# LepistaBioinformatics/classeq2

Hardware: AMD Instinct MI355X
Metric: query placements/sec, 10k-leaf tree, 150 bp reads (higher is better)
Workload: dtype u64

## Files before the change

classeq2_amd/csrc/cls_api.cpp:

```cpp
#include <hip/hip_runtime.h>
#include <ctype.h>
#include <stdio.h>
#include <stdlib.h>
#include <string.h>

#include <algorithm>
#include <mutex>
#include <new>
#include <string>
#include <thread>
#include <vector>

#include "cls_db.h"
#include "cls_device.h"
#include "cls_kernels.h"
#include "cls_place.h"
#include "cls_tally.h"
#include "cls_tuning.h"

namespace {

thread_local std::string g_err;

int fail(int code, const std::string& msg) {
// ... 74 lines not shown
    std::vector<CallSlot> calls;
    struct TreeRow { uint64_t id; uint32_t pre, size; };
    std::vector<TreeRow> tree_rows;
};

namespace cls {
Tuning& tuning() {
    static Tuning t;
    return t;
}
}
namespace {
struct Knob { const char* name; int cls::Tuning::*field; };
const Knob KNOBS[] = {
    {"no_fast", &cls::Tuning::no_fast}, {"no_order", &cls::Tuning::no_order}, {"force_list", &cls::Tuning::force_list},
    {"no_mask_halves", &cls::Tuning::no_mask_halves}, {"no_fat_direct", &cls::Tuning::no_fat_direct}, {"no_tile", &cls::Tuning::no_tile}, {"tile_pass_codes", &cls::Tuning::tile_pass_codes}, {"tile_set_words", &cls::Tuning::tile_set_words}, {"time_class", &cls::Tuning::time_class}, {"tile_one_per_cu", &cls::Tuning::tile_one_per_cu}, {"tile_min_kmers", &cls::Tuning::tile_min_kmers}, {"no_tile_order", &cls::Tuning::no_tile_order}, {"tile_deal", &cls::Tuning::tile_deal}, {"blocks_per_cu", &cls::Tuning::blocks_per_cu}, {"key_blocks_per_cu", &cls::Tuning::key_blocks_per_cu},
    {"long_blocks_per_cu", &cls::Tuning::long_blocks_per_cu}, {"order_mode", &cls::Tuning::order_mode},
    {"order_windows", &cls::Tuning::order_windows}, {"order_both_strands", &cls::Tuning::order_both_strands},
    {"order_block_shift", &cls::Tuning::order_block_shift}, {"order_sample_shift", &cls::Tuning::order_sample_shift},
    {"profile_stop", &cls::Tuning::profile_stop}, {"timing", &cls::Tuning::timing},
    {"build_full_key", &cls::Tuning::build_full_key}, {"tally_no_wave_combine", &cls::Tuning::tally_no_wave_combine},
};
}

extern "C" int cls_set_tuning(const char* name, int value) {
    if (!name) return fail(CLS_E_INVALID_ARG, "cls_set_tuning: null name");
    for (const Knob& k : KNOBS)
        if (strcmp(k.name, name) == 0) { cls::tuning().*(k.field) = value; return CLS_OK; }
    return fail(CLS_E_INVALID_ARG, std::string("cls_set_tuning: unknown knob ") + name);
}

// ... 102 lines not shown
    v.mz_bucket = (const uint32_t*)db->d_mz_bucket;
    v.direct = (const uint32_t*)db->d_direct;
    v.direct16 = (const uint32_t*)db->d_direct16;
    v.sets = (const cls::SetRec*)db->d_sets;
    v.sets2 = (const cls::SetRec*)db->d_sets2;
    v.table_mask = E.table.size() - 1;
    v.n_nodes = (uint32_t)E.nodes.size();
    v.n_buckets = (uint32_t)E.bucket_key.size();
    v.k = E.k;
    v.m_eff = E.m_eff;
    v.max_nonleaf_arity = E.max_nonleaf_arity;
    v.format = E.format;
    v.binary_tree = E.strictly_binary ? 1u : 0u;
    v.canonical = E.canonical ? 1u : 0u;
    v.n_sets = (uint32_t)E.sets.size();
    v.set_bits = 1;
    while (v.set_bits < 32 && (1ull << v.set_bits) < (uint64_t)E.sets.size()) ++v.set_bits;
    v.addr32 = (E.postings.size() * 4 < (1ull << 32) && E.direct.size() * 4 < (1ull << 32) && E.sets.size() * sizeof(cls::SetRec) < (1ull << 32)) ? 1u : 0u;
    cls_db_info& i = db->info;
    i.n_nodes = v.n_nodes;
    i.max_depth = E.max_depth;
    i.max_nonleaf_arity = E.max_nonleaf_arity;
    i.k_size = E.k;
    i.m_size = E.m;
    i.n_buckets = n_buckets;
    i.n_kmers = E.n_kmers;
    i.n_closed_kmers = E.n_closed;
    i.table_slots = E.table.size();
    i.postings_words = E.postings.size();
    i.hbm_bytes = E.nodes.size() * sizeof(cls::DNode) + E.table.size() * sizeof(cls::Slot) + (E.postings.size() + E.postings2.size()) * 4 + E.bucket_key.size() * 8 + E.mz_bucket.size() * 4 + E.direct.size() * 4 + E.direct16.size() * 4 + (E.sets.size() + E.sets2.size()) * sizeof(cls::SetRec);
// ... 998 lines not shown
```

classeq2_amd/csrc/cls_db.cpp:

```cpp
#include "cls_db.h"

#include "cls_murmur.h"
#include "cls_tuning.h"

#include <stdio.h>
#include <stdlib.h>
#include <string.h>

#include <algorithm>
#include <atomic>
#include <chrono>
#include <exception>
#include <functional>
#include <mutex>
#include <thread>

namespace cls {

namespace {

struct WorkerError {
    std::mutex mu;
    std::exception_ptr first;
    void capture() { std::lock_guard<std::mutex> g(mu); if (!first) first = std::current_exception(); }
// ... 336 lines not shown
        parallel_chunks(NK, nt, [&](unsigned, uint64_t lo, uint64_t hi) {
            for (uint64_t j = lo; j < hi; ++j) set_of[j] = rank[tmp_set[j]] + 1;
        });
        std::vector<uint32_t>().swap(tmp_set);
        std::vector<uint32_t>().swap(rank);
        E.n_sets = NS;
        lap("set order");
        std::vector<uint64_t> set_rec(NS + 1);
        uint64_t n_recs = 1;
        for (uint64_t g = 0; g < NS; ++g) { set_rec[g] = n_recs; n_recs += keys[g].n ? keys[g].n - 1 : 0; }
        set_rec[NS] = n_recs;
        if (n_recs >= (1ULL << 32)) { err = "split trees exceed 2^32 records"; return CLS_E_BAD_DB; }
        HugeVec<uint32_t> recs((n_recs + 1) * 4, 0);
        recs[2] = 0xFFFFFFFFu;
        const bool mask_halves = !tuning().no_mask_halves;
        HugeVec<uint32_t> recs2(mask_halves ? (n_recs + 1) * 4 : 0, 0);
        if (mask_halves) { recs2[2] = 0xFFFFFFFFu; set_mask.assign(NS + 1, 0u); }
        E.sets.assign(NS + 1, SetRec{0u, 0xFFFFFFFFu, 0u, 0u});
        parallel_chunks(NS, nt, [&](unsigned, uint64_t lo, uint64_t hi) {
            std::vector<uint32_t> dd, stk, L, R, pos, span_lo, span_hi;
            for (uint64_t g = lo; g < hi; ++g) {
                const uint32_t* w = words_of(keys[g].rep);
                const uint32_t n = w[0] & POST_LEN_MASK;
                const uint32_t* tip = w + POST_HEADER_WORDS;
                const uint64_t base = set_rec[g];
                dd.assign(n, 0); L.assign(n, 0); R.assign(n, 0);
                for (uint32_t i = 1; i < n; ++i) {
                    uint32_t a = tip[i - 1];
                    while (!(tip[i] < a + size_by_pre[a])) a = parent_pre[a];
                    dd[i] = depth_by_pre[a];
// ... 23 lines not shown
                        if (left_heavy) { if (r) stk.push_back(r); if (l) stk.push_back(l); }
                        else { if (l) stk.push_back(l); if (r) stk.push_back(r); }
                    }
                }
                auto at = [&](uint32_t i) { return (uint32_t)(base + pos[i]); };
                for (uint32_t i = 1; i < n; ++i) {
                    uint32_t* t = &recs[(size_t)at(i) * 4];
                    t[0] = tip[i - 1];
                    t[1] = L[i] ? at(L[i]) : 0;
                    t[2] = tip[i];
                    t[3] = R[i] ? at(R[i]) : 0;
                    if (mask_halves) {
                        uint32_t* u = &recs2[(size_t)at(i) * 4];
                        u[0] = t[0]; u[1] = t[1]; u[2] = t[2]; u[3] = t[3];
                        const uint32_t l0 = span_lo[i], r1 = span_hi[i];
                        if (tip[i - 1] - tip[l0] < MASK_HALF_SPAN) {
                            uint32_t bits = 0;
                            for (uint32_t j = l0; j < i; ++j) bits |= 1u << (tip[j] - tip[l0]);
                            u[0] = tip[i - 1] | MASK_HALF; u[1] = bits;
                        }
                        if (tip[r1 - 1] - tip[i] < MASK_HALF_SPAN) {
                            uint32_t bits = 0;
                            for (uint32_t j = i; j < r1; ++j) bits |= 1u << (tip[j] - tip[i]);
                            u[2] = tip[i] | MASK_HALF; u[3] = bits;
                        }
                    }
                }
                if (mask_halves && n && tip[n - 1] - tip[0] < MASK_HALF_SPAN) {
                    uint32_t bits = 0;
                    for (uint32_t j = 0; j < n; ++j) bits |= 1u << (tip[j] - tip[0]);
                    set_mask[g + 1] = bits;
                }
                uint32_t lg = 0;
                while (lg < 31 && (1u << lg) <= n) ++lg;
                SetRec& sr = E.sets[g + 1];
                sr.x = root ? at(root) : 0;
                sr.vlo_lg = n ? ((lg << DIRECT_TIP_BITS) | tip[0]) : 0xFFFFFFFFu;
                sr.vhi_root = (n ? tip[n - 1] : 0u) | ((w[0] & POST_HAS_ROOT) ? 0x80000000u : 0u);
                sr.n_leaf = w[1];
// ... 127 lines not shown
                if (it != by_key.end()) E.mz_bucket[code] = it->second;
            }
        }
    }
    E.k = (uint32_t)d->k_size;
    E.m = (uint32_t)std::min<uint64_t>(d->m_size, UINT32_MAX);
    E.m_eff = (uint32_t)std::min<uint64_t>(d->m_size, d->k_size);
    E.n_kmers = NK;
    E.n_closed = n_closed.load();
    E.root_has_children = d->nodes[0].has_children != 0;
    return CLS_OK;
}

}

extern "C" int cls_db_debug_mask_halves(const cls_db_desc* d, uint64_t* counts) {
    try {
        cls::EncodedDb E;
        std::string err;
        const int rc = cls::encode_db(d, E, err);
        if (rc != CLS_OK) return rc;
        using namespace cls;
        counts[0] = counts[1] = counts[2] = 0;
        if (E.format != FMT_SPLIT || E.postings2.empty()) return CLS_OK;
        if (E.postings2.size() != E.postings.size()) return CLS_E_INTERNAL;
        const TipRec* recs = reinterpret_cast<const TipRec*>(E.postings.data());
        const TipRec* rec2 = reinterpret_cast<const TipRec*>(E.postings2.data());
        const uint64_t n_recs = E.postings.size() / 4;
        std::function<void(uint32_t, uint32_t, int, std::vector<uint32_t>&)> part = [&](uint32_t end_tip, uint32_t x, int side, std::vector<uint32_t>& out) {
            if (!x) { out.push_back(end_tip); return; }
            const TipRec& t = recs[x];
            part(t.tip_prev, t.l, 0, out);
            part(t.tip, t.r, 1, out);
            (void)side;
        };
        std::vector<uint32_t> tips;
        for (uint64_t x = 1; x + 1 < n_recs; ++x) {
            const TipRec& t = recs[x];
            const TipRec& u = rec2[x];
            if (t.tip_prev == 0 && t.tip == 0 && t.l == 0 && t.r == 0) continue;
            ++counts[0];
            for (int side = 0; side < 2; ++side) {
                const uint32_t end_tip = side ? t.tip : t.tip_prev, sub = side ? t.r : t.l;
                const uint32_t uw = side ? u.tip : u.tip_prev, ux = side ? u.r : u.l;
                tips.clear();
                part(end_tip, sub, side, tips);
                if (!std::is_sorted(tips.begin(), tips.end()) || (side ? tips.front() : tips.back()) != end_tip) return CLS_E_INTERNAL;
                const bool narrow = tips.back() - tips.front() < MASK_HALF_SPAN;
                if (uw & MASK_HALF) {
                    uint32_t bits = 0;
                    for (uint32_t v : tips) bits |= 1u << (v - tips.front());
                    if (!narrow || (uw & ~MASK_HALF) != end_tip || ux != bits) return CLS_E_INTERNAL;
                    ++counts[1];
                } else {
                    if (narrow || uw != end_tip || ux != sub) return CLS_E_INTERNAL;
                    ++counts[2];
                }
            }
        }
        return CLS_OK;
    } catch (const std::bad_alloc&) {
        return CLS_E_NOMEM;
    } catch (...) {
        return CLS_E_INTERNAL;
    }
}

extern "C" int cls_db_debug_members(const cls_db_desc* d, const uint64_t* hashes, const uint64_t* clade_ids, uint64_t n, uint8_t* out) {
    try {
        cls::EncodedDb E;
        std::string err;
        const int rc = cls::encode_db(d, E, err);
        if (rc != CLS_OK) return rc;
        using namespace cls;
        std::vector<std::pair<uint64_t, uint32_t>> id2row(E.nodes.size());
        for (uint32_t r = 0; r < E.nodes.size(); ++r) id2row[r] = {E.nodes[r].id, r};
        std::sort(id2row.begin(), id2row.end());
        const uint64_t mask = E.table.size() - 1;
        std::vector<uint32_t> tips, stk;
        for (uint64_t i = 0; i < n; ++i) {
            auto it = std::lower_bound(id2row.begin(), id2row.end(), std::make_pair(clade_ids[i], (uint32_t)0));
// ... 55 lines not shown
```

classeq2_amd/csrc/cls_db.h:

```cpp
#pragma once
#include <stdlib.h>
#include <sys/mman.h>

#include <new>
#include <string>
#include <vector>

#include "cls_device.h"

namespace cls {

constexpr uint64_t MAX_K = 1024;

template <class T>
struct HugeAlloc {
    using value_type = T;
    HugeAlloc() = default;
    template <class U> HugeAlloc(const HugeAlloc<U>&) {}
    T* allocate(size_t n) {
        const size_t bytes = n * sizeof(T);
        if (bytes < (8u << 20)) { void* p = malloc(bytes ? bytes : 1); if (!p) throw std::bad_alloc(); return static_cast<T*>(p); }
        const size_t huge = 2u << 20, padded = (bytes + huge - 1) & ~(huge - 1);
        void* p = aligned_alloc(huge, padded);
        if (!p) throw std::bad_alloc();
// ... 13 lines not shown
    HugeVec<Slot> table;
    HugeVec<uint32_t> postings2;
    HugeVec<uint32_t> postings;
    uint32_t format = FMT_LIST;
    bool strictly_binary = false;
    bool canonical = false;
    std::vector<uint64_t> bucket_key;
    std::vector<uint32_t> mz_bucket;
    HugeVec<SetRec> sets;
    HugeVec<SetRec> sets2;
    HugeVec<uint32_t> direct;
    HugeVec<uint32_t> direct16;
    uint32_t k = 0, m = 0, m_eff = 0;
    uint32_t max_depth = 0, max_nonleaf_arity = 0;
    uint64_t n_kmers = 0, n_closed = 0;
    uint64_t n_sets = 0;
    bool root_has_children = false;
};

int encode_db(const cls_db_desc* d, EncodedDb& E, std::string& err);

}
```

classeq2_amd/csrc/cls_device.h:

```cpp
#pragma once
#include <stdint.h>

#include "cls_place.h"

namespace cls {

struct DNode {
    uint32_t pre;
    uint32_t size;
    uint32_t first_child;
    uint32_t n_nonleaf;
    uint64_t id;
    uint32_t split;
    uint32_t flags;
};
static_assert(sizeof(DNode) == 32, "DNode");

struct Slot {
    uint64_t hash;
    uint64_t loc;
};
static_assert(sizeof(Slot) == 16, "Slot");
constexpr uint64_t SLOT_EMPTY = ~0ULL;
struct TSlot {
// ... 22 lines not shown
};
static_assert(sizeof(SetRec) == 16, "SetRec");
constexpr uint32_t DIRECT_MAX_K = 15;
constexpr uint32_t FAT_DIRECT_MAX_K = 12;
constexpr uint32_t DIRECT_TIP_BITS = 27;
constexpr uint32_t DIRECT_TIP_MASK = (1u << DIRECT_TIP_BITS) - 1;
struct TipRec {
    uint32_t tip_prev;
    uint32_t l;
    uint32_t tip;
    uint32_t r;
};
static_assert(sizeof(TipRec) == 16, "TipRec");
constexpr uint32_t MASK_HALF = 0x80000000u;
constexpr uint32_t MASK_HALF_SPAN = 32;
constexpr uint32_t FAT_X_IS_BITS = 0x40000000u;

enum : uint32_t { FMT_LIST = 0, FMT_SPLIT = 1 };

struct DbDev {
    const DNode* nodes;
    const uint32_t* kids;
    const Slot* table;
    const uint32_t* postings;
    const uint32_t* postings2;
    const uint64_t* bucket_key;
    const uint32_t* mz_bucket;
    const uint32_t* direct;
    const uint32_t* direct16;
    const SetRec* sets;
    const SetRec* sets2;
    uint64_t table_mask;
    uint32_t n_nodes;
    uint32_t n_buckets;
    uint32_t k;
    uint32_t m_eff;
    uint32_t max_nonleaf_arity;
    uint32_t format;
    uint32_t addr32;
    uint32_t binary_tree;
    uint32_t canonical;
    uint32_t set_bits;
    uint32_t n_sets;
};

struct PlaceParams {
    int32_t max_iterations;
    uint32_t remove_intersection;
    double min_match_coverage;
};

constexpr uint32_t MAX_READ_KMERS = 64 * 8 * 16;

}
```

classeq2_amd/csrc/cls_kernels.hip:

```cpp
#include <hip/hip_runtime.h>
#include <stdlib.h>

#include <algorithm>
#include <type_traits>

#include "cls_device.h"
#include "cls_devutil.h"
#include "cls_kernels.h"
#include "cls_murmur.h"
#include "cls_sort.h"
#include "cls_tuning.h"

namespace cls {

namespace {

constexpr int WAVES_PER_BLOCK = 4;
#ifndef MIN_WAVES_PER_EU
#define MIN_WAVES_PER_EU 4
#endif
#ifndef FAST_MIN_WAVES
#define FAST_MIN_WAVES 5
#endif
#ifndef CLS_NARROW_CANON_BITS
// ... 814 lines not shown
    typedef __attribute__((address_space(4))) const uint32_t as4_u32;
    as4_u32* p = (as4_u32*)(uintptr_t)(kids + 4 * (size_t)__builtin_amdgcn_readfirstlane(row));
    skids_t r;
#pragma unroll
    for (int i = 0; i < 4; ++i) r.s[i] = p[i];
    return r;
}

struct FastCtx {
    uint8_t* ascii;
    uint32_t* packed;
    uint32_t* set;
    uint32_t* gkey;
    uint32_t* gcnt;
    uint4* stage;
    uint32_t* ccnt;
    uint32_t* conly;
    uint32_t* cpre;
};
constexpr int FAST_SLOTS_NARROW = 5;
constexpr uint32_t FAST_MAX_ARITY = 256;

struct FatRec { uint32_t x, vlo_lg, vhi_root; };
template <int SET_BITS>
__device__ __forceinline__ void clear_tables(const FastCtx& cx, uint32_t table_bits, uint32_t lane) {
    if constexpr (SET_BITS == 0) {
        if (lane == 0) cx.set[0] = SET_EMPTY;
    } else {
        const uint4 ones = make_uint4(SET_EMPTY, SET_EMPTY, SET_EMPTY, SET_EMPTY), zero = make_uint4(0, 0, 0, 0);
        uint4* const s4 = reinterpret_cast<uint4*>(cx.set);
// ... 137 lines not shown
        key[s] = slot;
        kw[s] = (hit && ok) ? 1u : 0u;
    }
    return true;
}

constexpr uint32_t GRP_INACTIVE = 0x7FFFFFFFu;
__device__ __forceinline__ uint32_t mask_lt(uint32_t a, uint32_t b) { return (uint32_t)((int32_t)(a - b) >> 31); }
__device__ __forceinline__ uint32_t sign_mask(uint32_t d) {
    uint32_t m;
    asm("v_ashrrev_i32_e32 %0, 31, %1" : "=v"(m) : "v"(d));
    return m;
}
__device__ __forceinline__ uint32_t bfi(uint32_t m, uint32_t a, uint32_t b) { return (a & m) | (b & ~m); }

template <bool ADDR32, bool POLY, bool STATS, bool MANY, bool REG2>
__device__ __forceinline__ void descend_groups(const DbDev& db, const PlaceParams& prm, const FastCtx& cx, uint32_t n_sets, snode_t P,
                                               uint32_t r, cls_placement* __restrict__ out, uint32_t& ib) {
    const uint32_t lane = threadIdx.x & 63;
    const uint32_t n_chunks = uniform((n_sets + 63) >> 6);
    if (n_sets + lane < 64 * n_chunks) cx.stage[n_sets + lane] = uint4{GRP_INACTIVE, 0u, 0u, 0u};
    wave_sync();
    uint32_t vlo, vhi, x, wt;
    uint32_t vlo2, vhi2, x2, wt2;
    {
        const uint4 g = n_chunks ? cx.stage[lane] : uint4{GRP_INACTIVE, 0u, 0u, 0u};
        vlo = g.x; vhi = g.y; x = g.z; wt = g.w;
        const uint4 g2 = (REG2 && n_chunks > 1) ? cx.stage[64 + lane] : uint4{GRP_INACTIVE, 0u, 0u, 0u};
        vlo2 = g2.x; vhi2 = g2.y; x2 = g2.z; wt2 = g2.w;
    }
    constexpr uint32_t CL = REG2 ? 2u : 1u;
    const uint32_t n_loop = MANY ? n_chunks : 0u;
    uint32_t w_all = (wt & 0xFFFFFFu) + (wt2 & 0xFFFFFFu);
#pragma unroll 1
    for (uint32_t c = CL; c < n_loop; ++c) w_all += cx.stage[c * 64 + lane].w & 0xFFFFFFu;
    w_all = wave_sum(w_all);
    constexpr bool MASKS = true;
    const uint32_t* __restrict__ half = (MASKS && db.postings2) ? db.postings2 : db.postings;
    auto next_part = [&](uint32_t bound, uint32_t& v, uint32_t& xx, bool& bits) {
        if (MASKS && bits) {
            const uint32_t up = xx >> ((bound - v) & 31u);
            const uint32_t z = (uint32_t)__ffs((int)up) - 1u;
            v = bound + z; xx = up >> (z & 31u);
        } else {
            const uint2 t = ld_half<ADDR32>(half, xx, 1u);
            if (STATS) ib += 8;
            v = t.x & ~MASK_HALF; xx = t.y;
            if (MASKS) bits = (t.x & MASK_HALF) != 0u;
        }
    };
    const bool rm = prm.remove_intersection != 0;
    skids_t K{};
    if (POLY) K = load_kids(db.kids, 0);
    int32_t iteration = 0;
    for (;;) {
        ++iteration;
        if (iteration > prm.max_iterations) { write_record(out, r, CLS_ERR_MAX_ITER, 0, 0, (uint32_t)iteration, 0); return; }
        const uint32_t fc = P.s[2], m = P.s[3];
        if (POLY && (P.s[7] >> 8) != 2) {
            const DNode* __restrict__ nodes = db.nodes;
            uint32_t n_pass = 0, n_best = 0, best_row = 0;
            int32_t best_one = 0, best_rest = 0, best_diff = 0;
            if (m <= 4) {
                const uint32_t B0 = P.s[0] + 1, B1 = P.s[6], B2 = K.s[0], B3 = K.s[1], B4 = K.s[2];
                const uint32_t last_end = m == 0 ? B0 : m == 1 ? B1 : m == 2 ? B2 : m == 3 ? B3 : B4;
                uint32_t cA = 0, cB = 0, oA = 0, oB = 0, u_lane = 0;
                auto walk4 = [&](uint32_t v, uint32_t vh, uint32_t xx, uint32_t wf) {
                    uint32_t nin = 0, which = 0;
                    bool bits = (wf >> 31) != 0u;
                    const uint32_t w = wf & 0xFFFFFFu;
                    while (v < last_end) {
                        const uint32_t c = (v >= B1 ? 1u : 0u) + (v >= B2 ? 1u : 0u) + (v >= B3 ? 1u : 0u);
                        const uint32_t c_end = c == 0 ? B1 : c == 1 ? B2 : c == 2 ? B3 : B4;
                        const uint32_t inc = w << (16 * (c & 1u));
                        if (c < 2) cA += inc; else cB += inc;
                        if (nin == 0) which = c;
                        if (nin < 2) ++nin;
                        if (vh < c_end) break;
                        next_part(c_end, v, xx, bits);
                    }
                    if (nin == 1) { const uint32_t inc = w << (16 * (which & 1u)); if (which < 2) oA += inc; else oB += inc; }
                    u_lane += nin ? w : 0u;
                };
                walk4(vlo, vhi, x, wt);
                if (REG2) walk4(vlo2, vhi2, x2, wt2);
#pragma unroll 1
                for (uint32_t c = CL; c < n_loop; ++c) { const uint4 g = cx.stage[c * 64 + lane]; walk4(g.x, g.y, g.z, g.w); }
                cA = wave_sum(cA); cB = wave_sum(cB); oA = wave_sum(oA); oB = wave_sum(oB);
                const uint32_t U = wave_sum(u_lane);
#pragma unroll
                for (uint32_t ci = 0; ci < 4; ++ci) {
                    if (ci >= m) break;
                    const uint32_t cn = ((ci < 2 ? cA : cB) >> (16 * (ci & 1u))) & 0xFFFFu, on = ((ci < 2 ? oA : oB) >> (16 * (ci & 1u))) & 0xFFFFu;
                    if (!cn) continue;
                    const int32_t one = (int32_t)(rm ? on : cn), rest = (int32_t)(rm ? U - cn : U - on);
                    if (one <= rest) continue;
                    const int32_t diff = one - rest;
                    if (n_pass == 0 || diff > best_diff) { best_diff = diff; n_best = 1; best_row = fc + ci; best_one = one; best_rest = rest; }
                    else if (diff == best_diff) ++n_best;
                    ++n_pass;
                }
            } else {
                uint32_t last_end = 0;
                if (m) { const snode_t Lc = load_node(nodes, fc + m - 1); last_end = Lc.s[0] + Lc.s[1]; }
                if (STATS && lane == 0 && m) ib += 32;
                for (uint32_t i = lane; i < m; i += 64) { cx.ccnt[i] = 0; cx.conly[i] = 0; cx.cpre[i] = nodes[fc + i].pre; if (STATS) ib += 4; }
                if (lane == 0) cx.cpre[m] = last_end;
                wave_sync();
                uint32_t u_lane = 0;
                auto walk = [&](uint32_t v, uint32_t vh, uint32_t xx, uint32_t wf) {
                    uint32_t nin = 0, which = 0;
                    bool bits = (wf >> 31) != 0u;
                    const uint32_t w = wf & 0xFFFFFFu;
                    while (v < last_end) {
                        uint32_t lo_ = 0, hi_ = m;
                        while (hi_ - lo_ > 1) { const uint32_t mid = (lo_ + hi_) >> 1; if (cx.cpre[mid] <= v) lo_ = mid; else hi_ = mid; }
                        const uint32_t c_end = cx.cpre[lo_ + 1];
                        atomicAdd(&cx.ccnt[lo_], w);
                        if (nin == 0) which = lo_;
                        if (nin < 2) ++nin;
                        if (vh < c_end) break;
                        next_part(c_end, v, xx, bits);
                    }
                    if (nin == 1) atomicAdd(&cx.conly[which], w);
                    u_lane += nin ? w : 0u;
                };
                walk(vlo, vhi, x, wt);
                if (REG2) walk(vlo2, vhi2, x2, wt2);
#pragma unroll 1
                for (uint32_t c = CL; c < n_loop; ++c) { const uint4 g = cx.stage[c * 64 + lane]; walk(g.x, g.y, g.z, g.w); }
                const uint32_t U = wave_sum(u_lane);
                wave_sync();
                for (uint32_t base = 0; base < m; base += 64) {
                    const uint32_t ci = base + lane;
                    bool pass = false;
                    int32_t one = 0, rest = 0;
                    if (ci < m) {
                        const uint32_t cn = cx.ccnt[ci], on = cx.conly[ci];
                        if (cn) { one = (int32_t)(rm ? on : cn); rest = (int32_t)(rm ? U - cn : U - on); pass = one > rest; }
                    }
                    uint64_t pm = __ballot(pass);
                    while (pm) {
                        const int src = __ffsll((unsigned long long)pm) - 1;
                        const int32_t o1 = __shfl(one, src), r1 = __shfl(rest, src);
                        const int32_t diff = o1 - r1;
// ... 8 lines not shown
            const uint64_t pid = ((uint64_t)P.s[5] << 32) | P.s[4];
            if (n_pass == 0) {
                if (iteration == 1) write_record(out, r, CLS_UNCLASSIFIABLE_LEVEL1, 0, 0, 1, 0);
                else write_record(out, r, CLS_MAX_RESOLUTION, 0, 0, (uint32_t)iteration, pid);
                return;
            }
            if (n_pass > 1 && n_best != 1) { write_record(out, r, CLS_INCONCLUSIVE, (int32_t)n_pass, 0, (uint32_t)iteration, pid); return; }
            P = load_node(nodes, best_row);
            K = load_kids(db.kids, best_row);
            if (STATS && lane == 0) ib += 32;
            if (P.s[3] == 0) {
                write_record(out, r, CLS_IDENTITY_FOUND, best_one, best_rest, (uint32_t)iteration, ((uint64_t)P.s[5] << 32) | P.s[4]);
                return;
            }
            const uint32_t c0 = P.s[0], c_end = c0 + P.s[1];
            auto enter = [&](uint32_t& v, uint32_t& vh, uint32_t& xx, uint32_t& wf) {
                bool dead = v > vh;
                bool bits = (wf >> 31) != 0u;
                while (!dead && v < c0) {
                    if (vh < c0) { dead = true; break; }
                    next_part(bits ? c0 : 0u, v, xx, bits);
                }
                if (!dead && v < c_end && v != c0) {
                    if (vh >= c_end) {
                        if (MASKS && bits) { xx &= (1u << ((c_end - v) & 31u)) - 1u; vh = v + 31u - (uint32_t)__clz((int)xx); }
                        else {
                            const uint2 t = ld_half<ADDR32>(half, xx, 0u);
                            if (STATS) ib += 8;
                            vh = t.x & ~MASK_HALF; xx = t.y;
                            if (MASKS) bits = (t.x & MASK_HALF) != 0u;
                        }
                    }
                } else { v = GRP_INACTIVE; vh = 0; }
                if (MASKS) wf = (wf & 0xFFFFFFu) | (bits ? MASK_HALF : 0u);
            };
            enter(vlo, vhi, x, wt);
            if (REG2) enter(vlo2, vhi2, x2, wt2);
#pragma unroll 1
            for (uint32_t c = CL; c < n_loop; ++c) {
                uint4 g = cx.stage[c * 64 + lane];
                enter(g.x, g.y, g.z, g.w);
                cx.stage[c * 64 + lane] = g;
            }
            continue;
        }
        const uint32_t a0 = P.s[0] + 1, a1 = P.s[6];
        const uint32_t a1_lo = m == 0 ? 0u : a1, a1_hi = m < 2 ? GRP_INACTIVE : a1;
        uint32_t acc = 0;
        auto count = [&](uint32_t lo_, uint32_t hi_, uint32_t w) { acc += __umul24(w, ((lo_ - a1_lo) >> 31) + ((hi_ - a1_hi) >> 31)); };
        count(vlo, vhi, wt);
        if (REG2) count(vlo2, vhi2, wt2);
#pragma unroll 1
        for (uint32_t c = CL; c < n_loop; ++c) { const uint4 g = cx.stage[c * 64 + lane]; count(g.x, g.y, g.w); }
        const int32_t diff_ab = (int32_t)(wave_sum(acc) - w_all);
        auto final_counts = [&](uint32_t& cnt_a, uint32_t& cnt_b, uint32_t& both) {
            uint32_t ca = 0, cb = 0, bo = 0;
            auto count3 = [&](uint32_t lo_, uint32_t hi_, uint32_t w) {
// ... 32 lines not shown
                         ((uint64_t)P.s[5] << 32) | P.s[4]);
            return;
        }
        auto narrow_side = [&](auto side) {
            constexpr bool RIGHT = decltype(side)::value;
            auto classify = [&](uint32_t lo_, uint32_t hi_, uint32_t w_, uint32_t& strm, uint32_t& rd, uint32_t& aux) {
                const uint32_t lt = sign_mask(lo_ - a1), nge = sign_mask(hi_ - a1);
                if (!RIGHT) { aux = lt & sign_mask(a0 - lo_); strm = aux & ~nge; }
                else { aux = nge; strm = lt & ~nge; }
                rd = MASKS ? (strm & ~sign_mask(w_)) : strm;
                if (STATS) ib += rd & 8u;
            };
            auto request = [&](uint32_t x_, uint32_t rd) -> uint2 {
                return ld_half<ADDR32>(half, x_ & rd, (RIGHT ? 1u : 0u) & rd);
            };
            auto finish = [&](uint32_t& lo_, uint32_t& hi_, uint32_t& x_, uint32_t& w_, uint32_t strm, uint32_t rd, uint32_t aux, uint2 t) {
                uint32_t end = t.x, xn = t.y;
                if (MASKS) {
                    w_ |= t.x & rd & MASK_HALF;
                    end &= ~MASK_HALF;
                    const uint32_t d = a1 - lo_;
                    uint32_t mend, mx;
                    if (!RIGHT) { mx = x_ & ((1u << (d & 31u)) - 1u); mend = lo_ + 31u - (uint32_t)__clz((int)mx); }
                    else { const uint32_t up = x_ >> (d & 31u); const uint32_t z = (uint32_t)__ffs((int)up) - 1u; mx = up >> (z & 31u); mend = a1 + z; }
                    end = bfi(rd, end, mend);
                    xn = bfi(rd, xn, mx);
                }
                x_ = bfi(strm, xn, x_);
                uint32_t keep;
                if (!RIGHT) {
                    keep = aux;
                    hi_ = bfi(strm, end, hi_);
                } else {
                    lo_ = bfi(strm, end, lo_);
                    keep = sign_mask(a1 - lo_) & ~aux;
                }
                lo_ = bfi(keep, lo_, GRP_INACTIVE);
                hi_ &= keep;
            };
            uint32_t s0 = 0, s1 = 0, r0 = 0, r1 = 0, k0 = 0, k1 = 0;
            uint2 t0{}, t1{};
            classify(vlo, vhi, wt, s0, r0, k0);
            if (REG2) classify(vlo2, vhi2, wt2, s1, r1, k1);
            if (!MASKS || __builtin_amdgcn_ballot_w64((r0 | r1) != 0u) != 0ull) {
                t0 = request(x, r0);
                if (REG2) t1 = request(x2, r1);
                __builtin_amdgcn_sched_barrier(0);
            }
            finish(vlo, vhi, x, wt, s0, r0, k0, t0);
            if (REG2) finish(vlo2, vhi2, x2, wt2, s1, r1, k1, t1);
#pragma unroll 1
            for (uint32_t c = CL; c < n_loop; ++c) {
                uint4 g = cx.stage[c * 64 + lane];
                uint32_t sm, rm_, km;
                classify(g.x, g.y, g.w, sm, rm_, km);
                const uint2 t = request(g.z, rm_);
                finish(g.x, g.y, g.z, g.w, sm, rm_, km, t);
                cx.stage[c * 64 + lane] = g;
            }
        };
        if (right) narrow_side(std::true_type{}); else narrow_side(std::false_type{});
    }
}

template <int SLOTS, int SET_BITS, bool STATS, bool ADDR32, int MODE, bool POLY>
__device__ __forceinline__ void place_read_fast(const DbDev& db, const PlaceParams& prm, const FastCtx& cx,
                                                const uint8_t* __restrict__ bases, uint64_t b0, uint64_t b1, uint32_t r,
                                                cls_placement* __restrict__ out, cls_query_stats* __restrict__ stats,
                                                uint32_t profile_stop_arg) {
#ifdef CLS_PROFILE_HOOKS
    const uint32_t profile_stop = profile_stop_arg;
#else
    constexpr uint32_t profile_stop = 0;
// ... 137 lines not shown
    if constexpr (!POLY) in_registers = uniform(n_sets) <= 128;
    constexpr bool REG2 = !POLY || MODE != 2;
    if (in_registers) descend_groups<ADDR32, POLY, STATS, false, REG2>(db, prm, cx, n_sets, P, r, out, ib);
    else descend_groups<ADDR32, POLY, STATS, true, REG2>(db, prm, cx, n_sets, P, r, out, ib);
    put_index_bytes();
}

template <int SLOTS, int SET_BITS, bool STATS, bool ADDR32, int MODE, bool POLY>
__global__ __launch_bounds__(64 * WAVES_PER_BLOCK, SLOTS > 5 ? FAST_MIN_WAVES_WIDE : POLY ? FAST_MIN_WAVES_POLY : FAST_MIN_WAVES) void place_fast_kernel(
    DbDev db, PlaceParams prm, const uint8_t* __restrict__ bases, const uint64_t* __restrict__ offsets,
    const uint32_t* __restrict__ list, const uint32_t* __restrict__ list_len, uint32_t list_n, uint32_t xcd_chunks,
    cls_placement* __restrict__ out, cls_query_stats* __restrict__ stats, uint32_t ascii_cap, uint32_t profile_stop) {
    extern __shared__ __align__(16) uint8_t smem[];
    const uint32_t wave = threadIdx.x >> 6;
    const uint32_t packed_words = MODE == 2 ? 0u : ((ascii_cap >> 4) + 2 + 3) & ~3u;
    constexpr bool FITS = (12u << SET_BITS) >= 16u * 64 * ((MODE == 1 || MODE == 4) ? (SLOTS + 1) / 2 : SLOTS);
    if constexpr (FITS) {
    const uint32_t per_wave = ascii_cap + 4u * packed_words + (12u << SET_BITS) + (POLY ? 12u * FAST_MAX_ARITY + 16u : 0u);
    FastCtx cx;
    cx.ascii = smem + wave * per_wave;
    cx.packed = reinterpret_cast<uint32_t*>(cx.ascii + ascii_cap);
    cx.set = cx.packed + packed_words;
    cx.gkey = cx.set + (1u << SET_BITS);
    cx.gcnt = cx.gkey + (1u << SET_BITS);
    cx.stage = reinterpret_cast<uint4*>(cx.set);
    cx.ccnt = cx.gcnt + (1u << SET_BITS);
    cx.conly = cx.ccnt + FAST_MAX_ARITY;
    cx.cpre = cx.conly + FAST_MAX_ARITY;
    if (xcd_chunks && SLOTS > FAST_SLOTS_NARROW && *list_len == 0) return;
    const uint32_t n_list = xcd_chunks ? list_n : *list_len;
    const uint32_t xcd = blockIdx.x & 7u, bpx = gridDim.x >> 3;
    const uint32_t chunk = xcd_chunks ? (n_list + 7u) >> 3 : n_list;
    const uint32_t first = xcd_chunks ? (blockIdx.x >> 3) * WAVES_PER_BLOCK + wave : blockIdx.x * WAVES_PER_BLOCK + wave;
    const uint32_t stride = (xcd_chunks ? bpx : gridDim.x) * WAVES_PER_BLOCK;
    const uint32_t origin = xcd_chunks ? xcd * chunk : 0u;
    constexpr uint32_t cap = 64 * SLOTS;
    for (uint32_t ql = first; ql < chunk; ql += stride) {
        const uint32_t q = origin + ql;
        if (q >= n_list) break;
        const uint32_t r = list[q];
// ... 945 lines not shown
```

classeq2_amd/csrc/cls_tuning.h:

```cpp
#pragma once

namespace cls {

struct Tuning {
    int no_fast = 0;
    int no_order = 0;
    int force_list = 0;
    int no_mask_halves = 0;
    int no_fat_direct = 0;
    int no_tile = 0;
    int tile_pass_codes = 0;
    int tile_set_words = 0;
    int tile_min_kmers = 0;
    int tile_deal = 64;
    int no_tile_order = 0;
    int tile_one_per_cu = 0;
    int time_class = 0;
    int blocks_per_cu = 0;
    int key_blocks_per_cu = 0;
    int long_blocks_per_cu = 2;
    int order_mode = 0;
    int order_windows = 64;
    int order_both_strands = 0;
    int order_block_shift = 2;
// ... 11 lines not shown
```

Baseline: 158.5 million.

## Add optional 64-row bitmask encoding for split-tree half records

Adds a mask_rows knob (default 32) that can encode split-tree half records as 64-bit tip bitmasks instead of 32-bit ones. The right-side masks are stored bit-reversed so their end can be recovered with a leading-zero count. The device descent code now carries a high mask word through next_part, enter and finish, and stores it in a new per-lane shared-memory array. The aim is to replace more pointer-chasing record loads with register bit operations. In exchange, every path does wider 64-bit arithmetic and uses extra shared memory, which tightens the FITS condition even when the default 32-row mode is used.

```diff
diff --git a/classeq2_amd/csrc/cls_api.cpp b/classeq2_amd/csrc/cls_api.cpp
--- a/classeq2_amd/csrc/cls_api.cpp
+++ b/classeq2_amd/csrc/cls_api.cpp
@@ -112,7 +112,7 @@
 struct Knob { const char* name; int cls::Tuning::*field; };
 const Knob KNOBS[] = {
     {"no_fast", &cls::Tuning::no_fast}, {"no_order", &cls::Tuning::no_order}, {"force_list", &cls::Tuning::force_list},
-    {"no_mask_halves", &cls::Tuning::no_mask_halves}, {"no_fat_direct", &cls::Tuning::no_fat_direct}, {"no_tile", &cls::Tuning::no_tile}, {"tile_pass_codes", &cls::Tuning::tile_pass_codes}, {"tile_set_words", &cls::Tuning::tile_set_words}, {"time_class", &cls::Tuning::time_class}, {"tile_one_per_cu", &cls::Tuning::tile_one_per_cu}, {"tile_min_kmers", &cls::Tuning::tile_min_kmers}, {"no_tile_order", &cls::Tuning::no_tile_order}, {"tile_deal", &cls::Tuning::tile_deal}, {"blocks_per_cu", &cls::Tuning::blocks_per_cu}, {"key_blocks_per_cu", &cls::Tuning::key_blocks_per_cu},
+    {"no_mask_halves", &cls::Tuning::no_mask_halves}, {"mask_rows", &cls::Tuning::mask_rows}, {"no_fat_direct", &cls::Tuning::no_fat_direct}, {"no_tile", &cls::Tuning::no_tile}, {"tile_pass_codes", &cls::Tuning::tile_pass_codes}, {"tile_set_words", &cls::Tuning::tile_set_words}, {"time_class", &cls::Tuning::time_class}, {"tile_one_per_cu", &cls::Tuning::tile_one_per_cu}, {"tile_min_kmers", &cls::Tuning::tile_min_kmers}, {"no_tile_order", &cls::Tuning::no_tile_order}, {"tile_deal", &cls::Tuning::tile_deal}, {"blocks_per_cu", &cls::Tuning::blocks_per_cu}, {"key_blocks_per_cu", &cls::Tuning::key_blocks_per_cu},
     {"long_blocks_per_cu", &cls::Tuning::long_blocks_per_cu}, {"order_mode", &cls::Tuning::order_mode},
     {"order_windows", &cls::Tuning::order_windows}, {"order_both_strands", &cls::Tuning::order_both_strands},
     {"order_block_shift", &cls::Tuning::order_block_shift}, {"order_sample_shift", &cls::Tuning::order_sample_shift},
@@ -245,6 +245,7 @@
     v.binary_tree = E.strictly_binary ? 1u : 0u;
     v.canonical = E.canonical ? 1u : 0u;
     v.n_sets = (uint32_t)E.sets.size();
+    v.mask_rows = E.mask_rows;
     v.set_bits = 1;
     while (v.set_bits < 32 && (1ull << v.set_bits) < (uint64_t)E.sets.size()) ++v.set_bits;
     v.addr32 = (E.postings.size() * 4 < (1ull << 32) && E.direct.size() * 4 < (1ull << 32) && E.sets.size() * sizeof(cls::SetRec) < (1ull << 32)) ? 1u : 0u;
diff --git a/classeq2_amd/csrc/cls_db.cpp b/classeq2_amd/csrc/cls_db.cpp
--- a/classeq2_amd/csrc/cls_db.cpp
+++ b/classeq2_amd/csrc/cls_db.cpp
@@ -374,6 +374,9 @@
         HugeVec<uint32_t> recs((n_recs + 1) * 4, 0);
         recs[2] = 0xFFFFFFFFu;
         const bool mask_halves = !tuning().no_mask_halves;
+        if (mask_halves && tuning().mask_rows != 32 && tuning().mask_rows != 64) { err = "tuning knob mask_rows must be 32 or 64"; return CLS_E_INVALID_ARG; }
+        const bool rows64 = tuning().mask_rows == 64;
+        E.mask_rows = mask_halves ? (rows64 ? MASK_HALF_SPAN64 : MASK_HALF_SPAN) : 0u;
         HugeVec<uint32_t> recs2(mask_halves ? (n_recs + 1) * 4 : 0, 0);
         if (mask_halves) { recs2[2] = 0xFFFFFFFFu; set_mask.assign(NS + 1, 0u); }
         E.sets.assign(NS + 1, SetRec{0u, 0xFFFFFFFFu, 0u, 0u});
@@ -427,15 +430,29 @@
                         uint32_t* u = &recs2[(size_t)at(i) * 4];
                         u[0] = t[0]; u[1] = t[1]; u[2] = t[2]; u[3] = t[3];
                         const uint32_t l0 = span_lo[i], r1 = span_hi[i];
-                        if (tip[i - 1] - tip[l0] < MASK_HALF_SPAN) {
-                            uint32_t bits = 0;
-                            for (uint32_t j = l0; j < i; ++j) bits |= 1u << (tip[j] - tip[l0]);
-                            u[0] = tip[i - 1] | MASK_HALF; u[1] = bits;
-                        }
-                        if (tip[r1 - 1] - tip[i] < MASK_HALF_SPAN) {
-                            uint32_t bits = 0;
-                            for (uint32_t j = i; j < r1; ++j) bits |= 1u << (tip[j] - tip[i]);
-                            u[2] = tip[i] | MASK_HALF; u[3] = bits;
+                        if (rows64) {
+                            auto put = [&](uint32_t* h, uint64_t m) { h[0] = MASK_HALF | (uint32_t)((m >> 1) & 0x7FFFFFFFu); h[1] = (uint32_t)(m >> 32); };
+                            if (tip[i - 1] - tip[l0] < MASK_HALF_SPAN64) {
+                                uint64_t m = 0;
+                                for (uint32_t j = l0; j < i; ++j) m |= 1ull << (tip[j] - tip[l0]);
+                                put(u, m);
+                            }
+                            if (tip[r1 - 1] - tip[i] < MASK_HALF_SPAN64) {
+                                uint64_t m = 0;
+                                for (uint32_t j = i; j < r1; ++j) m |= 1ull << (tip[r1 - 1] - tip[j]);
+                                put(u + 2, m);
+                            }
+                        } else {
+                            if (tip[i - 1] - tip[l0] < MASK_HALF_SPAN) {
+                                uint32_t bits = 0;
+                                for (uint32_t j = l0; j < i; ++j) bits |= 1u << (tip[j] - tip[l0]);
+                                u[0] = tip[i - 1] | MASK_HALF; u[1] = bits;
+                            }
+                            if (tip[r1 - 1] - tip[i] < MASK_HALF_SPAN) {
+                                uint32_t bits = 0;
+                                for (uint32_t j = i; j < r1; ++j) bits |= 1u << (tip[j] - tip[i]);
+                                u[2] = tip[i] | MASK_HALF; u[3] = bits;
+                            }
                         }
                     }
                 }
@@ -593,7 +610,7 @@
 
 }
 
-extern "C" int cls_db_debug_mask_halves(const cls_db_desc* d, uint64_t* counts) {
+static int debug_mask_halves(const cls_db_desc* d, uint64_t* counts, uint64_t* spans) {
     try {
         cls::EncodedDb E;
         std::string err;
@@ -601,17 +618,19 @@
         if (rc != CLS_OK) return rc;
         using namespace cls;
         counts[0] = counts[1] = counts[2] = 0;
+        if (spans) std::fill(spans, spans + 4 * 129, 0ull);
         if (E.format != FMT_SPLIT || E.postings2.empty()) return CLS_OK;
         if (E.postings2.size() != E.postings.size()) return CLS_E_INTERNAL;
+        if (E.mask_rows != MASK_HALF_SPAN && E.mask_rows != MASK_HALF_SPAN64) return CLS_E_INTERNAL;
+        const bool rows64 = E.mask_rows == MASK_HALF_SPAN64;
         const TipRec* recs = reinterpret_cast<const TipRec*>(E.postings.data());
         const TipRec* rec2 = reinterpret_cast<const TipRec*>(E.postings2.data());
         const uint64_t n_recs = E.postings.size() / 4;
-        std::function<void(uint32_t, uint32_t, int, std::vector<uint32_t>&)> part = [&](uint32_t end_tip, uint32_t x, int side, std::vector<uint32_t>& out) {
+        std::function<void(uint32_t, uint32_t, std::vector<uint32_t>&)> part = [&](uint32_t end_tip, uint32_t x, std::vector<uint32_t>& out) {
             if (!x) { out.push_back(end_tip); return; }
             const TipRec& t = recs[x];
-            part(t.tip_prev, t.l, 0, out);
-            part(t.tip, t.r, 1, out);
-            (void)side;
+            part(t.tip_prev, t.l, out);
+            part(t.tip, t.r, out);
         };
         std::vector<uint32_t> tips;
         for (uint64_t x = 1; x + 1 < n_recs; ++x) {
@@ -623,18 +642,31 @@
                 const uint32_t end_tip = side ? t.tip : t.tip_prev, sub = side ? t.r : t.l;
                 const uint32_t uw = side ? u.tip : u.tip_prev, ux = side ? u.r : u.l;
                 tips.clear();
-                part(end_tip, sub, side, tips);
+                part(end_tip, sub, tips);
                 if (!std::is_sorted(tips.begin(), tips.end()) || (side ? tips.front() : tips.back()) != end_tip) return CLS_E_INTERNAL;
-                const bool narrow = tips.back() - tips.front() < MASK_HALF_SPAN;
-                if (uw & MASK_HALF) {
-                    uint32_t bits = 0;
-                    for (uint32_t v : tips) bits |= 1u << (v - tips.front());
-                    if (!narrow || (uw & ~MASK_HALF) != end_tip || ux != bits) return CLS_E_INTERNAL;
+                const uint32_t rows = tips.back() - tips.front() + 1;
+                const bool narrow = rows <= E.mask_rows;
+                const bool is_mask = (uw & MASK_HALF) != 0;
+                if (is_mask) {
+                    if (!narrow) return CLS_E_INTERNAL;
+                    if (rows64) {
+                        uint64_t m = 0;
+                        for (uint32_t v : tips) m |= 1ull << (side ? tips.back() - v : v - tips.front());
+                        if (uw != (MASK_HALF | (uint32_t)((m >> 1) & 0x7FFFFFFFu)) || ux != (uint32_t)(m >> 32)) return CLS_E_INTERNAL;
+                        const uint64_t back = ((uint64_t)ux << 32) | ((uint64_t)(uw << 1)) | 1ull;
+                        const uint32_t top = 63u - (uint32_t)__builtin_clzll(back);
+                        if (back != m || (side ? tips.back() - top != tips.front() : tips.front() + top != tips.back())) return CLS_E_INTERNAL;
+                    } else {
+                        uint32_t bits = 0;
+                        for (uint32_t v : tips) bits |= 1u << (v - tips.front());
+                        if ((uw & ~MASK_HALF) != end_tip || ux != bits) return CLS_E_INTERNAL;
+                    }
                     ++counts[1];
                 } else {
                     if (narrow || uw != end_tip || ux != sub) return CLS_E_INTERNAL;
                     ++counts[2];
                 }
+                if (spans) ++spans[(side * 2 + (is_mask ? 1 : 0)) * 129 + std::min<uint32_t>(rows, 128u)];
             }
         }
         return CLS_OK;
@@ -644,6 +676,8 @@
         return CLS_E_INTERNAL;
     }
 }
+extern "C" int cls_db_debug_mask_halves(const cls_db_desc* d, uint64_t* counts) { return debug_mask_halves(d, counts, nullptr); }
+extern "C" int cls_db_debug_mask_spans(const cls_db_desc* d, uint64_t* counts, uint64_t* spans) { return debug_mask_halves(d, counts, spans); }
 
 extern "C" int cls_db_debug_members(const cls_db_desc* d, const uint64_t* hashes, const uint64_t* clade_ids, uint64_t n, uint8_t* out) {
     try {
diff --git a/classeq2_amd/csrc/cls_db.h b/classeq2_amd/csrc/cls_db.h
--- a/classeq2_amd/csrc/cls_db.h
+++ b/classeq2_amd/csrc/cls_db.h
@@ -51,6 +51,7 @@
     uint32_t k = 0, m = 0, m_eff = 0;
     uint32_t max_depth = 0, max_nonleaf_arity = 0;
     uint64_t n_kmers = 0, n_closed = 0;
+    uint32_t mask_rows = 0;
     uint64_t n_sets = 0;
     bool root_has_children = false;
 };
diff --git a/classeq2_amd/csrc/cls_device.h b/classeq2_amd/csrc/cls_device.h
--- a/classeq2_amd/csrc/cls_device.h
+++ b/classeq2_amd/csrc/cls_device.h
@@ -60,6 +60,7 @@
 static_assert(sizeof(TipRec) == 16, "TipRec");
 constexpr uint32_t MASK_HALF = 0x80000000u;
 constexpr uint32_t MASK_HALF_SPAN = 32;
+constexpr uint32_t MASK_HALF_SPAN64 = 64;
 constexpr uint32_t FAT_X_IS_BITS = 0x40000000u;
 
 enum : uint32_t { FMT_LIST = 0, FMT_SPLIT = 1 };
@@ -88,6 +89,7 @@
     uint32_t canonical;
     uint32_t set_bits;
     uint32_t n_sets;
+    uint32_t mask_rows;
 };
 
 struct PlaceParams {
diff --git a/classeq2_amd/csrc/cls_kernels.hip b/classeq2_amd/csrc/cls_kernels.hip
--- a/classeq2_amd/csrc/cls_kernels.hip
+++ b/classeq2_amd/csrc/cls_kernels.hip
@@ -852,6 +852,7 @@
     uint32_t* gkey;
     uint32_t* gcnt;
     uint4* stage;
+    uint32_t* xh;
     uint32_t* ccnt;
     uint32_t* conly;
     uint32_t* cpre;
@@ -1019,6 +1020,15 @@
 }
 __device__ __forceinline__ uint32_t bfi(uint32_t m, uint32_t a, uint32_t b) { return (a & m) | (b & ~m); }
 
+__device__ __forceinline__ uint64_t bits64(uint32_t lo_word, uint32_t hi_word) { return ((uint64_t)hi_word << 32) | lo_word; }
+template <bool RIGHT>
+__device__ __forceinline__ void mask64_arrive(uint2 t, uint32_t lo, uint32_t hi, uint64_t& m, uint32_t& end) {
+    const uint64_t a = bits64((t.x << 1) | 1u, t.y);
+    const uint32_t lz = (uint32_t)__clzll((long long)a);
+    if (!RIGHT) { m = a; end = lo + (63u - lz); }
+    else { m = __builtin_bitreverse64(a) >> lz; end = hi - (63u - lz); }
+}
+
 template <bool ADDR32, bool POLY, bool STATS, bool MANY, bool REG2>
 __device__ __forceinline__ void descend_groups(const DbDev& db, const PlaceParams& prm, const FastCtx& cx, uint32_t n_sets, snode_t P,
                                                uint32_t r, cls_placement* __restrict__ out, uint32_t& ib) {
@@ -1028,6 +1038,7 @@
     wave_sync();
     uint32_t vlo, vhi, x, wt;
     uint32_t vlo2, vhi2, x2, wt2;
+    uint32_t xh = 0, xh2 = 0;
     {
         const uint4 g = n_chunks ? cx.stage[lane] : uint4{GRP_INACTIVE, 0u, 0u, 0u};
         vlo = g.x; vhi = g.y; x = g.z; wt = g.w;
@@ -1036,22 +1047,30 @@
     }
     constexpr uint32_t CL = REG2 ? 2u : 1u;
     const uint32_t n_loop = MANY ? n_chunks : 0u;
+#pragma unroll 1
+    for (uint32_t c = CL; c < n_loop; ++c) cx.xh[(c - 1) * 64 + lane] = 0u;
     uint32_t w_all = (wt & 0xFFFFFFu) + (wt2 & 0xFFFFFFu);
 #pragma unroll 1
     for (uint32_t c = CL; c < n_loop; ++c) w_all += cx.stage[c * 64 + lane].w & 0xFFFFFFu;
     w_all = wave_sum(w_all);
+    const bool rows64 = db.mask_rows == MASK_HALF_SPAN64;
     constexpr bool MASKS = true;
     const uint32_t* __restrict__ half = (MASKS && db.postings2) ? db.postings2 : db.postings;
-    auto next_part = [&](uint32_t bound, uint32_t& v, uint32_t& xx, bool& bits) {
+    auto next_part = [&](uint32_t bound, uint32_t& v, uint32_t vh, uint32_t& xx, uint32_t& xxh, bool& bits) {
         if (MASKS && bits) {
-            const uint32_t up = xx >> ((bound - v) & 31u);
-            const uint32_t z = (uint32_t)__ffs((int)up) - 1u;
-            v = bound + z; xx = up >> (z & 31u);
+            const uint64_t up = bits64(xx, xxh) >> ((bound - v) & 63u);
+            const uint32_t z = (uint32_t)__ffsll((long long)up) - 1u;
+            const uint64_t mx = up >> (z & 63u);
+            v = bound + z; xx = (uint32_t)mx; xxh = (uint32_t)(mx >> 32);
         } else {
             const uint2 t = ld_half<ADDR32>(half, xx, 1u);
             if (STATS) ib += 8;
-            v = t.x & ~MASK_HALF; xx = t.y;
             if (MASKS) bits = (t.x & MASK_HALF) != 0u;
+            if (MASKS && rows64 && bits) {
+                uint64_t mx;
+                mask64_arrive<true>(t, v, vh, mx, v);
+                xx = (uint32_t)mx; xxh = (uint32_t)(mx >> 32);
+            } else { v = t.x & ~MASK_HALF; xx = t.y; xxh = 0u; }
         }
     };
     const bool rm = prm.remove_intersection != 0;
@@ -1070,7 +1089,7 @@
                 const uint32_t B0 = P.s[0] + 1, B1 = P.s[6], B2 = K.s[0], B3 = K.s[1], B4 = K.s[2];
                 const uint32_t last_end = m == 0 ? B0 : m == 1 ? B1 : m == 2 ? B2 : m == 3 ? B3 : B4;
                 uint32_t cA = 0, cB = 0, oA = 0, oB = 0, u_lane = 0;
-                auto walk4 = [&](uint32_t v, uint32_t vh, uint32_t xx, uint32_t wf) {
+                auto walk4 = [&](uint32_t v, uint32_t vh, uint32_t xx, uint32_t xxh, uint32_t wf) {
                     uint32_t nin = 0, which = 0;
                     bool bits = (wf >> 31) != 0u;
                     const uint32_t w = wf & 0xFFFFFFu;
@@ -1082,15 +1101,15 @@
                         if (nin == 0) which = c;
                         if (nin < 2) ++nin;
                         if (vh < c_end) break;
-                        next_part(c_end, v, xx, bits);
+                        next_part(c_end, v, vh, xx, xxh, bits);
                     }
                     if (nin == 1) { const uint32_t inc = w << (16 * (which & 1u)); if (which < 2) oA += inc; else oB += inc; }
                     u_lane += nin ? w : 0u;
                 };
-                walk4(vlo, vhi, x, wt);
-                if (REG2) walk4(vlo2, vhi2, x2, wt2);
+                walk4(vlo, vhi, x, xh, wt);
+                if (REG2) walk4(vlo2, vhi2, x2, xh2, wt2);
 #pragma unroll 1
-                for (uint32_t c = CL; c < n_loop; ++c) { const uint4 g = cx.stage[c * 64 + lane]; walk4(g.x, g.y, g.z, g.w); }
+                for (uint32_t c = CL; c < n_loop; ++c) { const uint4 g = cx.stage[c * 64 + lane]; walk4(g.x, g.y, g.z, cx.xh[(c - 1) * 64 + lane], g.w); }
                 cA = wave_sum(cA); cB = wave_sum(cB); oA = wave_sum(oA); oB = wave_sum(oB);
                 const uint32_t U = wave_sum(u_lane);
 #pragma unroll
@@ -1113,7 +1132,7 @@
                 if (lane == 0) cx.cpre[m] = last_end;
                 wave_sync();
                 uint32_t u_lane = 0;
-                auto walk = [&](uint32_t v, uint32_t vh, uint32_t xx, uint32_t wf) {
+                auto walk = [&](uint32_t v, uint32_t vh, uint32_t xx, uint32_t xxh, uint32_t wf) {
                     uint32_t nin = 0, which = 0;
                     bool bits = (wf >> 31) != 0u;
                     const uint32_t w = wf & 0xFFFFFFu;
@@ -1125,15 +1144,15 @@
                         if (nin == 0) which = lo_;
                         if (nin < 2) ++nin;
                         if (vh < c_end) break;
-                        next_part(c_end, v, xx, bits);
+                        next_part(c_end, v, vh, xx, xxh, bits);
                     }
                     if (nin == 1) atomicAdd(&cx.conly[which], w);
                     u_lane += nin ? w : 0u;
                 };
-                walk(vlo, vhi, x, wt);
-                if (REG2) walk(vlo2, vhi2, x2, wt2);
+                walk(vlo, vhi, x, xh, wt);
+                if (REG2) walk(vlo2, vhi2, x2, xh2, wt2);
 #pragma unroll 1
-                for (uint32_t c = CL; c < n_loop; ++c) { const uint4 g = cx.stage[c * 64 + lane]; walk(g.x, g.y, g.z, g.w); }
+                for (uint32_t c = CL; c < n_loop; ++c) { const uint4 g = cx.stage[c * 64 + lane]; walk(g.x, g.y, g.z, cx.xh[(c - 1) * 64 + lane], g.w); }
                 const uint32_t U = wave_sum(u_lane);
                 wave_sync();
                 for (uint32_t base = 0; base < m; base += 64) {
@@ -1172,33 +1191,42 @@
                 return;
             }
             const uint32_t c0 = P.s[0], c_end = c0 + P.s[1];
-            auto enter = [&](uint32_t& v, uint32_t& vh, uint32_t& xx, uint32_t& wf) {
+            auto enter = [&](uint32_t& v, uint32_t& vh, uint32_t& xx, uint32_t& xxh, uint32_t& wf) {
                 bool dead = v > vh;
                 bool bits = (wf >> 31) != 0u;
                 while (!dead && v < c0) {
                     if (vh < c0) { dead = true; break; }
-                    next_part(bits ? c0 : 0u, v, xx, bits);
+                    next_part(bits ? c0 : 0u, v, vh, xx, xxh, bits);
                 }
                 if (!dead && v < c_end && v != c0) {
                     if (vh >= c_end) {
-                        if (MASKS && bits) { xx &= (1u << ((c_end - v) & 31u)) - 1u; vh = v + 31u - (uint32_t)__clz((int)xx); }
-                        else {
+                        if (MASKS && bits) {
+                            const uint64_t mx = bits64(xx, xxh) & ((1ull << ((c_end - v) & 63u)) - 1ull);
+                            xx = (uint32_t)mx; xxh = (uint32_t)(mx >> 32);
+                            vh = v + 63u - (uint32_t)__clzll((long long)mx);
+                        } else {
                             const uint2 t = ld_half<ADDR32>(half, xx, 0u);
                             if (STATS) ib += 8;
-                            vh = t.x & ~MASK_HALF; xx = t.y;
                             if (MASKS) bits = (t.x & MASK_HALF) != 0u;
+                            if (MASKS && rows64 && bits) {
+                                uint64_t mx;
+                                mask64_arrive<false>(t, v, vh, mx, vh);
+                                xx = (uint32_t)mx; xxh = (uint32_t)(mx >> 32);
+                            } else { vh = t.x & ~MASK_HALF; xx = t.y; xxh = 0u; }
                         }
                     }
                 } else { v = GRP_INACTIVE; vh = 0; }
                 if (MASKS) wf = (wf & 0xFFFFFFu) | (bits ? MASK_HALF : 0u);
             };
-            enter(vlo, vhi, x, wt);
-            if (REG2) enter(vlo2, vhi2, x2, wt2);
+            enter(vlo, vhi, x, xh, wt);
+            if (REG2) enter(vlo2, vhi2, x2, xh2, wt2);
 #pragma unroll 1
             for (uint32_t c = CL; c < n_loop; ++c) {
                 uint4 g = cx.stage[c * 64 + lane];
-                enter(g.x, g.y, g.z, g.w);
+                uint32_t gh = cx.xh[(c - 1) * 64 + lane];
+                enter(g.x, g.y, g.z, gh, g.w);
                 cx.stage[c * 64 + lane] = g;
+                cx.xh[(c - 1) * 64 + lane] = gh;
             }
             continue;
         }
@@ -1261,18 +1289,33 @@
             auto request = [&](uint32_t x_, uint32_t rd) -> uint2 {
                 return ld_half<ADDR32>(half, x_ & rd, (RIGHT ? 1u : 0u) & rd);
             };
-            auto finish = [&](uint32_t& lo_, uint32_t& hi_, uint32_t& x_, uint32_t& w_, uint32_t strm, uint32_t rd, uint32_t aux, uint2 t) {
-                uint32_t end = t.x, xn = t.y;
+            auto finish = [&](uint32_t& lo_, uint32_t& hi_, uint32_t& x_, uint32_t& xh_, uint32_t& w_, uint32_t strm, uint32_t rd, uint32_t aux, uint2 t) {
+                uint32_t end = t.x & ~MASK_HALF, xn = t.y, xhn = 0u;
                 if (MASKS) {
                     w_ |= t.x & rd & MASK_HALF;
-                    end &= ~MASK_HALF;
-                    const uint32_t d = a1 - lo_;
-                    uint32_t mend, mx;
-                    if (!RIGHT) { mx = x_ & ((1u << (d & 31u)) - 1u); mend = lo_ + 31u - (uint32_t)__clz((int)mx); }
-                    else { const uint32_t up = x_ >> (d & 31u); const uint32_t z = (uint32_t)__ffs((int)up) - 1u; mx = up >> (z & 31u); mend = a1 + z; }
-                    end = bfi(rd, end, mend);
-                    xn = bfi(rd, xn, mx);
-                }
+                    const uint32_t arr = rows64 ? (sign_mask(t.x) & rd) : 0u;
+                    const uint32_t a_lo = (t.x << 1) | 1u;
+                    const uint32_t d = (a1 - lo_) & 63u;
+                    const uint64_t cur = bits64(x_, xh_);
+                    uint32_t mend;
+                    uint64_t mx;
+                    if (!RIGHT) {
+                        const uint64_t below = cur & ((1ull << d) - 1ull);
+                        mx = bits64(bfi(arr, a_lo, (uint32_t)below), bfi(arr, t.y, (uint32_t)(below >> 32)));
+                        mend = lo_ + 63u - (uint32_t)__clzll((long long)mx);
+                    } else {
+                        const uint64_t up = cur >> d;
+                        const uint64_t src = bits64(bfi(arr, __builtin_bitreverse32(t.y), (uint32_t)up), bfi(arr, __builtin_bitreverse32(a_lo), (uint32_t)(up >> 32)));
+                        const uint32_t z = (uint32_t)__ffsll((long long)src) - 1u;
+                        mx = src >> (z & 63u);
+                        mend = bfi(arr, hi_ - 63u, a1) + z;
+                    }
+                    const uint32_t from_bits = arr | ~rd;
+                    end = bfi(from_bits, mend, end);
+                    xn = bfi(from_bits, (uint32_t)mx, xn);
+                    xhn = (uint32_t)(mx >> 32) & from_bits;
+                }
+                xh_ = bfi(strm, xhn, xh_);
                 x_ = bfi(strm, xn, x_);
                 uint32_t keep;
                 if (!RIGHT) {
@@ -1294,16 +1337,18 @@
                 if (REG2) t1 = request(x2, r1);
                 __builtin_amdgcn_sched_barrier(0);
             }
-            finish(vlo, vhi, x, wt, s0, r0, k0, t0);
-            if (REG2) finish(vlo2, vhi2, x2, wt2, s1, r1, k1, t1);
+            finish(vlo, vhi, x, xh, wt, s0, r0, k0, t0);
+            if (REG2) finish(vlo2, vhi2, x2, xh2, wt2, s1, r1, k1, t1);
 #pragma unroll 1
             for (uint32_t c = CL; c < n_loop; ++c) {
                 uint4 g = cx.stage[c * 64 + lane];
+                uint32_t gh = cx.xh[(c - 1) * 64 + lane];
                 uint32_t sm, rm_, km;
                 classify(g.x, g.y, g.w, sm, rm_, km);
                 const uint2 t = request(g.z, rm_);
-                finish(g.x, g.y, g.z, g.w, sm, rm_, km, t);
+                finish(g.x, g.y, g.z, gh, g.w, sm, rm_, km, t);
                 cx.stage[c * 64 + lane] = g;
+                cx.xh[(c - 1) * 64 + lane] = gh;
             }
         };
         if (right) narrow_side(std::true_type{}); else narrow_side(std::false_type{});
@@ -1471,7 +1516,8 @@
     extern __shared__ __align__(16) uint8_t smem[];
     const uint32_t wave = threadIdx.x >> 6;
     const uint32_t packed_words = MODE == 2 ? 0u : ((ascii_cap >> 4) + 2 + 3) & ~3u;
-    constexpr bool FITS = (12u << SET_BITS) >= 16u * 64 * ((MODE == 1 || MODE == 4) ? (SLOTS + 1) / 2 : SLOTS);
+    constexpr uint32_t LSLOTS = (MODE == 1 || MODE == 4) ? (SLOTS + 1) / 2 : SLOTS;
+    constexpr bool FITS = (12u << SET_BITS) >= 16u * 64 * LSLOTS + 4u * 64 * (LSLOTS - 1);
     if constexpr (FITS) {
     const uint32_t per_wave = ascii_cap + 4u * packed_words + (12u << SET_BITS) + (POLY ? 12u * FAST_MAX_ARITY + 16u : 0u);
     FastCtx cx;
@@ -1481,6 +1527,7 @@
     cx.gkey = cx.set + (1u << SET_BITS);
     cx.gcnt = cx.gkey + (1u << SET_BITS);
     cx.stage = reinterpret_cast<uint4*>(cx.set);
+    cx.xh = reinterpret_cast<uint32_t*>(cx.stage + 64 * LSLOTS);
     cx.ccnt = cx.gcnt + (1u << SET_BITS);
     cx.conly = cx.ccnt + FAST_MAX_ARITY;
     cx.cpre = cx.conly + FAST_MAX_ARITY;
diff --git a/classeq2_amd/csrc/cls_tuning.h b/classeq2_amd/csrc/cls_tuning.h
--- a/classeq2_amd/csrc/cls_tuning.h
+++ b/classeq2_amd/csrc/cls_tuning.h
@@ -7,6 +7,7 @@
     int no_order = 0;
     int force_list = 0;
     int no_mask_halves = 0;
+    int mask_rows = 32;
     int no_fat_direct = 0;
     int no_tile = 0;
     int tile_pass_codes = 0;
```

Result: slower. 146.3 million (-7.7%).
